# SidRama/Longitudinal-VAE

Measured on AMD Instinct MI355X. Metric: ELBO-steps/sec (exact-KL L-VAE step, Health-MNIST N=4096 L=16), higher is better.
Workload: dtype f16x3-split (fp32-equivalent)

## Files before the change

### longitudinal-vae_amd/csrc/kl_hyper.hip

```cpp
#include "blkinv.hpp"
#include "gram_tab.hpp"
#include "prof.hpp"

namespace lvae {

constexpr int kHbMaxBin = 4;
constexpr int kHbBins = 128;
constexpr int kHbBins2 = 4096;
constexpr int kHbRun = 64;
constexpr int kHbSmall = 16;
constexpr int kHbSmallest = 4;
constexpr int kHbNear = 4;
constexpr int kHbBlk = 4;
constexpr int kHbT = 64;
constexpr int kHbTP = 68;
constexpr int kHbNB = 24;
constexpr int kHbNQ = kHbNB / 4;
constexpr int kHbNearS = 2 * kHbBins2;
constexpr int kHbNearK = kHbNearS + kHbNear + 1;
constexpr int kHbA = kHbNearK + kHbNear;
constexpr int kHbTail = 2 * kHbNear + 1 + kHbBins;
constexpr int kHbPart = 2 * kHbBins2 + kHbTail;

struct HbDev {
  int on, nbin, big, nbins, nb2, nnear;
  int gmin[kTabMaxBits], grng[kTabMaxBits];
  int wmin[kTabMaxG], wrng[kTabMaxG];
  int bmask[kHbMaxBin], bgrp[kHbMaxBin], boff[kHbMaxBin], bn[kHbMaxBin], b2off[kHbMaxBin];
  int cbin[LVAE_MAX_COMP];
  int nslot[kHbNear];
};

typedef unsigned hb_u32x4 __attribute__((ext_vector_type(4)));

struct HbWs {
  HbDev* dev;
  uint8_t* pbin;
  int* rs;
  int* re;
  double* part;
  float* tab;
  hb_u32x4* rkey;
  double* hscr;
  double* nscr;
  size_t bytes;
  HbWs(char* base, int np_, int L) {
    size_t off = 0;
    auto take = [&](size_t b) {
      char* p = base ? base + off : nullptr;
      off += align256(b);
      return p;
    };
    dev = (HbDev*)take(sizeof(HbDev));
    pbin = (uint8_t*)take((size_t)kHbMaxBin * np_);
    rs = (int*)take((size_t)np_ * sizeof(int));
    re = (int*)take((size_t)np_ * sizeof(int));
    part = (double*)take((size_t)L * (np_ / kHbT) * kHbPart * sizeof(double));
    tab = (float*)take((size_t)L * kTabMaxBwdLds * sizeof(float));
    rkey = (hb_u32x4*)take((size_t)np_ * sizeof(hb_u32x4));
    hscr = (double*)take((size_t)L * (np_ / kHbT) * kHbBins * kHbT * sizeof(double));
    nscr = (double*)take((size_t)L * (np_ / kHbT) * kHbNB * 256 * sizeof(double));
    bytes = off;
  }
};
size_t kl_hyper_bytes(int np_, int L) { return HbWs(nullptr, np_, L).bytes; }
HbDev* kl_hyper_dev(void* base, int np_, int L) { return HbWs((char*)base, np_, L).dev; }

__global__ __launch_bounds__(1024) void hb_plan_kernel(GramTab tb, const double* __restrict__ x, int ldx, int n,
                                                       int np_, const int* __restrict__ covflag, HbWs ws, int enable) {
  __shared__ int lo[kTabMaxBits + kTabMaxG], hi[kTabMaxBits + kTabMaxG];
  __shared__ int fail;
  __shared__ HbDev d;
  const int tid = threadIdx.x, nd = tb.nbits + tb.ng;
  if (*covflag != 2) {
    if (tid == 0) ws.dev->on = 0;
    return;
  }
  if (tid < kTabMaxBits + kTabMaxG) {
    lo[tid] = INT_MAX;
    hi[tid] = INT_MIN;
  }
  if (tid == 0) fail = 0;
  __syncthreads();
  for (int q = 0; q < nd; ++q) {
    const int dim = q < tb.nbits ? tb.bdim[q] : tb.gdim[q - tb.nbits];
    if (dim < 0) continue;
    int mn = INT_MAX, mx = INT_MIN;
    for (int i = tid; i < n; i += 1024) {
      const int v = (int)x[(int64_t)i * ldx + dim];
      mn = min(mn, v);
      mx = max(mx, v);
    }
#pragma unroll
    for (int o = 32; o > 0; o >>= 1) {
      mn = min(mn, __shfl_xor(mn, o, 64));
      mx = max(mx, __shfl_xor(mx, o, 64));
    }
    if ((tid & 63) == 0) {
      atomicMin(&lo[q], mn);
      atomicMax(&hi[q], mx);
    }
  }
  __syncthreads();
  if (tid == 0) {
    HbDev p{};
    int f = 0;
    p.big = -1;
    for (int b = 0; b < tb.nbits; ++b) {
      p.gmin[b] = lo[b];
      p.grng[b] = hi[b] - lo[b] + 1;
      if (tb.bkind[b] == LVAE_CAT && p.grng[b] > kHbSmallest && (p.big < 0 || p.grng[b] > p.grng[p.big])) p.big = b;
    }
    for (int b = 0; b < tb.nbits; ++b)
      if (b != p.big && tb.bkind[b] == LVAE_CAT && p.grng[b] > kHbSmall) f = 1;
    for (int g = 0; g < tb.ng; ++g) {
      p.wmin[g] = tb.gdim[g] >= 0 ? lo[tb.nbits + g] : 0;
      p.wrng[g] = tb.gdim[g] >= 0 ? hi[tb.nbits + g] - lo[tb.nbits + g] + 1 : 1;
    }
    for (int r = 0; r < tb.n_comp; ++r) {
      p.cbin[r] = -1;
      if (p.big >= 0 && ((tb.cmask[r] >> p.big) & 1)) continue;
      const int grp = tb.ckind[r] >= 0 ? tb.cgrp[r] : -1;
      int g = 0;
      while (g < p.nbin && !(p.bmask[g] == tb.cmask[r] && p.bgrp[g] == grp)) ++g;
      if (g == p.nbin) {
        if (p.nbin == kHbMaxBin) {
          f = 1;
          break;
        }
        long long nb = grp >= 0 ? p.wrng[grp] : 1;
        for (int b = 0; b < tb.nbits; ++b)
          if ((tb.cmask[r] >> b) & 1) nb *= p.grng[b];
        if (nb > kHbBins) {
          f = 1;
          break;
        }
        p.bmask[g] = tb.cmask[r];
        p.bgrp[g] = grp;
        p.bn[g] = (int)nb;
        p.boff[g] = p.nbins;
        p.b2off[g] = p.nb2;
        p.nbins += (int)nb;
        p.nb2 += (int)(nb * nb);
        ++p.nbin;
      }
      p.cbin[r] = g;
    }
    if (p.nbins > kHbBins || p.nb2 > kHbBins2) f = 1;
    {
      int nblk = 0;
      for (int g = 0; g < p.nbin; ++g) nblk += (p.bn[g] + 31) / 32;
      if (nblk > kHbBlk) f = 1;
    }
    for (int k = 0; k < tb.pbeg[tb.ng] && !f; ++k)
      if (p.cbin[tb.pcomp[tb.porder[k]]] < 0) {
        if (p.nnear == kHbNear) f = 1;
        else p.nslot[p.nnear++] = k;
      }
    d = p;
    fail = f;
  }
  __syncthreads();
  const int bd = d.big >= 0 ? tb.bdim[d.big] : -1;
  int bad = 0;
  for (int i = tid; i < np_; i += 1024) {
    int s = -1, e = -1;
    if (bd >= 0 && i < n) {
      const double v = x[(int64_t)i * ldx + bd];
      if (i > 0 && x[(int64_t)(i - 1) * ldx + bd] > v) bad = 1;
      s = i;
      while (s > 0 && i - s < kHbRun && x[(int64_t)(s - 1) * ldx + bd] == v) --s;
      e = i + 1;
      while (e < n && e - i < kHbRun && x[(int64_t)e * ldx + bd] == v) ++e;
      if (e - s > kHbRun || (s > 0 && x[(int64_t)(s - 1) * ldx + bd] == v) || (e < n && x[(int64_t)e * ldx + bd] == v))
        bad = 1;
    }
    ws.rs[i] = s;
    ws.re[i] = e;
    hb_u32x4 key = {0u, 0u, 0u, 0u};
    if (i < n) {
      for (int b = 0; b < tb.nbits; ++b) {
        const int xv = (int)x[(int64_t)i * ldx + tb.bdim[b]], v = xv - d.gmin[b];
        if (b == d.big) continue;
        if (tb.bkind[b] == LVAE_CAT) {
          if (v < 0 || v > 63) bad = 1;
          key.x |= (unsigned)(v & 63) << (6 * b);
        } else {
          if (xv != 0 && xv != 1) bad = 1;
          key.w |= (unsigned)(xv == 1) << b;
        }
      }
      for (int g = 0; g < tb.ng; ++g) {
        if (tb.gdim[g] < 0) continue;
        const int v = (int)x[(int64_t)i * ldx + tb.gdim[g]] - d.wmin[g];
        if (v < 0 || v > 65535) bad = 1;
        const unsigned u = (unsigned)(v & 0xffff);
        if (g == 0) key.y |= u;
        else if (g == 1) key.y |= u << 16;
        else key.z |= u;
      }
    }
    ws.rkey[i] = key;
    for (int g = 0; g < kHbMaxBin; ++g) {
      int idx = 255;
      if (g < d.nbin && i < n) {
        idx = 0;
        for (int b = 0; b < tb.nbits; ++b)
          if ((d.bmask[g] >> b) & 1) idx = idx * d.grng[b] + ((int)x[(int64_t)i * ldx + tb.bdim[b]] - d.gmin[b]);
        if (d.bgrp[g] >= 0) idx = idx * d.wrng[d.bgrp[g]] + ((int)x[(int64_t)i * ldx + tb.gdim[d.bgrp[g]]] - d.wmin[d.bgrp[g]]);
      }
      ws.pbin[(size_t)g * np_ + i] = (uint8_t)idx;
    }
  }
  if (__any(bad) && (tid & 63) == 0) atomicOr(&fail, 1);
  __syncthreads();
  if (tid == 0) {
    HbDev p = d;
    p.on = (!fail && enable) ? 1 : 0;
    *ws.dev = p;
  }
}


__global__ __launch_bounds__(256) void hb_tab_kernel(GramTab tb, HbWs ws, const double* __restrict__ params) {
  __shared__ float sp[64];
  const int tid = threadIdx.x, l = blockIdx.y, e = blockIdx.x * 256 + tid;
  if (!ws.dev->on) return;
  if (tid < tb.n_params) sp[tid] = float(params[(int64_t)l * tb.n_params + tid]);
  __syncthreads();
  if (e < tb.pbeg[tb.ng] * (1 << tb.nbits) * kTabR) ws.tab[(int64_t)l * kTabMaxBwdLds + e] = tab_bwd_entry(tb, sp, e);
}

__device__ inline unsigned hb_pair_code(hb_u32x4 ki, hb_u32x4 kj, unsigned catbits, int ng) {
  const unsigned x = ki.x ^ kj.x, x1 = x | (x >> 1), x3 = x1 | (x1 >> 2), x5 = x3 | (x1 >> 4);
  const unsigned fail = (((x5 & 0x1041041u) * 0x108421u) >> 20) & 31u;
  unsigned c = (catbits & ~fail) | (ki.w & kj.w);
  const unsigned a0 = ki.y & 0xffffu, b0 = kj.y & 0xffffu, a1 = ki.y >> 16, b1 = kj.y >> 16;
  const unsigned a2 = ki.z & 0xffffu, b2 = kj.z & 0xffffu;
  const unsigned d0 = a0 > b0 ? a0 - b0 : b0 - a0, d1 = a1 > b1 ? a1 - b1 : b1 - a1, d2 = a2 > b2 ? a2 - b2 : b2 - a2;
  const unsigned cap = (unsigned)kTabD;
  c |= (d0 < cap ? d0 : cap) << 8;
  if (ng > 1) c |= (d1 < cap ? d1 : cap) << 16;
  if (ng > 2) c |= (d2 < cap ? d2 : cap) << 24;
  return c;
}

__device__ inline unsigned hb_catbits(const GramTab& tb) {
  unsigned m = 0;
#pragma unroll
  for (int b = 0; b < kTabMaxBits; ++b)
    if (b < tb.nbits && tb.bkind[b] == LVAE_CAT) m |= 1u << b;
  return m;
}

__device__ inline void hb_near_tables(const GramTab& tb, const HbDev& d, const float* __restrict__ gt, int tstride,
                                      float* __restrict__ tab, int* __restrict__ sgrp) {
  const int tid = threadIdx.x;
  if (tid < d.nnear) sgrp[tid] = tb.cgrp[tb.pcomp[tb.porder[d.nslot[tid]]]];
  for (int e = tid; e < d.nnear * tstride; e += blockDim.x) tab[e] = gt[d.nslot[e / tstride] * tstride + e % tstride];
}

__device__ inline float hb_near_d(const float* tab, int tk, unsigned code, int grp) {
  return tab[tk + (int)(code & 0xffu) * kTabR + (int)((code >> (8 * (grp + 1))) & 0xffu)];
}

__global__ __launch_bounds__(256) void hb_near_kernel(GramTab tb, HbWs ws, int n, int np_,
                                                      const float* __restrict__ Kinv, const double* __restrict__ alpha) {
  __shared__ HbDev d;
  __shared__ int sgrp[kHbNear];
  __shared__ double red[4][kHbNear];
  extern __shared__ float ntab[];
  const int tid = threadIdx.x, lane = tid & 63, w = tid >> 6, I = blockIdx.x, l = blockIdx.y, I0 = I * kHbT;
  if (tid == 0) d = *ws.dev;
  __syncthreads();
  if (!d.on) return;
  const int tstride = (1 << tb.nbits) * kTabR, nnear = d.nnear;
  hb_near_tables(tb, d, ws.tab + (int64_t)l * kTabMaxBwdLds, tstride, ntab, sgrp);
  __syncthreads();
  const float* K = Kinv + (int64_t)l * np_ * np_;
  const double* al = alpha + (int64_t)l * np_;
  const unsigned catbits = hb_catbits(tb);
  double acc[kHbNear];
#pragma unroll
  for (int k = 0; k < kHbNear; ++k) acc[k] = 0.0;
  if (d.big >= 0) {
    for (int e = tid; e < kHbT * kHbRun; e += 256) {
      const int i = I0 + e / kHbRun, jj = e % kHbRun;
      if (i >= n) continue;
      const int s = ws.rs[i], len = ws.re[i] - s;
      if (jj >= len) continue;
      const int j = s + jj;
      const unsigned c = hb_pair_code(ws.rkey[i], ws.rkey[j], catbits, tb.ng);
      const double val = 0.5 * ((double)K[(int64_t)i * np_ + j] - al[i] * al[j]);
#pragma unroll
      for (int k = 0; k < kHbNear; ++k)
        if (k < nnear) acc[k] += val * (double)hb_near_d(ntab, k * tstride, c, sgrp[k]);
    }
  }
#pragma unroll
  for (int k = 0; k < kHbNear; ++k) {
    const double sk = wave_sum(acc[k]);
    if (lane == 0) red[w][k] = sk;
  }
  __syncthreads();
  if (tid < kHbNear)
    ws.part[((int64_t)l * (np_ / kHbT) + I) * kHbPart + kHbNearK + tid] =
        ((red[0][tid] + red[1][tid]) + red[2][tid]) + red[3][tid];
}


#ifdef LVAE_HB_STAMP
#define HB_STAMP(t)                                                                   \
  do {                                                                                \
    __builtin_amdgcn_sched_barrier(0);                                                \
    asm volatile("s_memtime %0\n\ts_waitcnt lgkmcnt(0)" : "=s"(t)::"memory");       \
    __builtin_amdgcn_sched_barrier(0);                                                \
  } while (0)
#else
#define HB_STAMP(t) \
  do {              \
  } while (0)
#endif

typedef float hb_f32x2 __attribute__((ext_vector_type(2)));
typedef float hb_f32x4 __attribute__((ext_vector_type(4)));
typedef float hb_f32x16 __attribute__((ext_vector_type(16)));
typedef __bf16 hb_bf16x8 __attribute__((ext_vector_type(8)));
typedef __bf16 hb_bf16x2 __attribute__((ext_vector_type(2)));
constexpr int kHbSlabThreads = 256, kHbSlabWaves = kHbSlabThreads / 64;
#ifndef LVAE_HB_FOLD
#define LVAE_HB_FOLD 16
#endif
constexpr int kHbFold = LVAE_HB_FOLD;
#ifndef LVAE_HB_DEPTH
#define LVAE_HB_DEPTH 1
#endif
constexpr int kHbDepth = LVAE_HB_DEPTH;
static_assert(kHbDepth == 1 || kHbDepth == 2 || kHbDepth == 4, "nt = np / 64 is a multiple of 4");

struct HbPre {
  hb_f32x2 pk[8];
  int pbn;
  hb_f32x4 vr[2];
};

__device__ inline unsigned hb_pk_bf16(float a, float b) {
  const hb_bf16x2 v = {(__bf16)a, (__bf16)b};
  return __builtin_bit_cast(unsigned, v);
}
__device__ inline float hb_bf_lo(unsigned u) { return __uint_as_float(u << 16); }
__device__ inline float hb_bf_hi(unsigned u) { return __uint_as_float(u & 0xffff0000u); }

__device__ inline int hb_pl_off(int c, int k) { return c * 32 + ((k ^ ((c >> 1) & 7)) << 2); }

__device__ inline void hb_split8(const float* a, hb_u32x4& hi, hb_u32x4& mid, hb_u32x4& lo) {
#pragma unroll
  for (int k = 0; k < 4; ++k) {
    const float x0 = a[2 * k], x1 = a[2 * k + 1];
    const unsigned h = hb_pk_bf16(x0, x1);
    const float r0 = x0 - hb_bf_lo(h), r1 = x1 - hb_bf_hi(h);
    const unsigned m = hb_pk_bf16(r0, r1);
    const float s0 = r0 - hb_bf_lo(m), s1 = r1 - hb_bf_hi(m);
    hi[k] = h;
    mid[k] = m;
    lo[k] = hb_pk_bf16(s0, s1);
  }
}

__global__ __launch_bounds__(kHbSlabThreads, 2) void hb_slab_kernel(GramTab tb, HbWs ws, int n, int np_,
                                                                    const float* __restrict__ Kinv,
                                                                    const float* __restrict__ vv,
                                                                    const double* __restrict__ alpha) {
  __shared__ HbDev d;
  __shared__ __attribute__((aligned(16))) float Tc[2 * kHbT * kHbTP];
  __shared__ __attribute__((aligned(16))) unsigned Pw[3][kHbT * 32];
  __shared__ __attribute__((aligned(8))) uint8_t rbin[kHbMaxBin][kHbT];
  __shared__ uint8_t cbin[kHbMaxBin][kHbT];
  __shared__ float vs[kHbT];
  __shared__ double acol[kHbT];
  __shared__ hb_u32x4 ckey[2 * kHbT];
  __shared__ int rstart[kHbT];
  __shared__ unsigned long long runends;
  __shared__ int nblk, nspan;
  __shared__ uint8_t blist[kHbNB];
  __shared__ int8_t blkid[64];
  __shared__ int sgrp[kHbNear];
  __shared__ int sbg[kHbBlk], sbb[kHbBlk], nbk;
  __shared__ double red[kHbSlabWaves][kHbNear + 1];
  extern __shared__ float tab[];
  const int tid = threadIdx.x, lane = tid & 63, w = tid >> 6, J = blockIdx.x, l = blockIdx.y, J0 = J * kHbT;
  if (tid == 0) d = *ws.dev;
  __syncthreads();
  if (!d.on) return;
  const int tstride = (1 << tb.nbits) * kTabR;
  if (tid < kHbT) {
    vs[tid] = vv[(int64_t)l * np_ + J0 + tid];
    acol[tid] = alpha[(int64_t)l * np_ + J0 + tid];
  }
  for (int e = tid; e < d.nbin * kHbT; e += kHbSlabThreads)
    cbin[e / kHbT][e % kHbT] = ws.pbin[(size_t)(e / kHbT) * np_ + J0 + e % kHbT];
  hb_near_tables(tb, d, ws.tab + (int64_t)l * kTabMaxBwdLds, tstride, tab, sgrp);
  if (tid < 2 * kHbT) {
    const int c = J0 - kHbT + tid;
    ckey[tid] = c >= 0 ? ws.rkey[c] : hb_u32x4{0u, 0u, 0u, 0u};
  }
  if (w == 0) {
    const int c = J0 + lane;
    const bool isend = d.big >= 0 && c < n && ws.re[c] == c + 1;
    const int s0 = isend ? ws.rs[c] : c;
    rstart[lane] = s0;
    const int ba = (s0 - J0 + kHbT) >> 4, bz = (c - J0 + kHbT) >> 4;
    unsigned long long m = 0;
    if (isend)
      for (int bi = ba; bi <= bz; ++bi)
        for (int bj = ba; bj <= bi; ++bj) m |= 1ull << (bi * 8 + bj);
#pragma unroll
    for (int o = 32; o > 0; o >>= 1) {
      const unsigned lo = __shfl_xor((unsigned)m, o, 64), hi = __shfl_xor((unsigned)(m >> 32), o, 64);
      m |= ((unsigned long long)hi << 32) | lo;
    }
    const unsigned long long ends = __ballot(isend), sp = __ballot(isend && s0 < J0);
    if (lane == 0) {
      runends = ends;
      nspan = sp != 0;
      int t = 0;
      for (int b = 0; b < 64; ++b) {
        blkid[b] = -1;
        if (((m >> b) & 1ull) && t < kHbNB) {
          blkid[b] = (int8_t)t;
          blist[t++] = (uint8_t)b;
        }
      }
      nblk = t;
    }
  }
  if (tid == 0) {
    int t = 0;
    for (int g = 0; g < d.nbin; ++g)
      for (int bb = 0; bb * 32 < d.bn[g] && t < kHbBlk; ++bb, ++t) {
        sbg[t] = g;
        sbb[t] = bb;
      }
    nbk = t;
  }
  __syncthreads();
  const float* K = Kinv + (int64_t)l * np_ * np_;
  const int nbin = d.nbin, nnear = d.nnear, nitem = 2 * nbk, nbl = nblk, span = nspan;
  const unsigned catbits = hb_catbits(tb);
  const int cb = w & 1, hh = lane >> 5, col = 32 * cb + (lane & 31);
  const int i0 = w, i1 = w + kHbSlabWaves;
  const bool it0 = i0 < nitem, it1 = i1 < nitem;
  int g0 = 0, b00 = 0, g1 = 0, b01 = 0;
  if (it0) {
    g0 = sbg[i0 >> 1];
    b00 = 32 * sbb[i0 >> 1];
  }
  if (it1) {
    g1 = sbg[i1 >> 1];
    b01 = 32 * sbb[i1 >> 1];
  }
  hb_f32x16 acc0 = {}, acc1 = {};
  double* Hs = ws.hscr + ((int64_t)l * (np_ / kHbT) + J) * kHbBins * kHbT;
  double* Ns = ws.nscr + ((int64_t)l * (np_ / kHbT) + J) * kHbNB * 256;
  const int li = lane & 15, lk = lane >> 4;
  bi_f32x4 nac[kHbNQ];
#pragma unroll
  for (int q = 0; q < kHbNQ; ++q) nac[q] = bi_f32x4{0.f, 0.f, 0.f, 0.f};
  double tS = 0.0;
  const int cp = tid & 31, i8 = tid >> 5;
  const float v0 = vs[2 * cp], v1 = vs[2 * cp + 1], r0 = sqrtf(v0), r1 = sqrtf(v1);
  const int nt = np_ / kHbT;

  auto fetch = [&](int I, HbPre& p) {
    const int I0 = I * kHbT;
#pragma unroll
    for (int u = 0; u < 8; ++u)
      p.pk[u] = __builtin_nontemporal_load(
          reinterpret_cast<const hb_f32x2*>(K + (int64_t)(I0 + 8 * i8 + u) * np_ + J0 + 2 * cp));
    p.pbn = (int)ws.pbin[(size_t)(w < nbin ? w : 0) * np_ + I0 + lane];
    const float* vr = vv + (int64_t)l * np_ + I0 + 8 * i8;
    p.vr[0] = *reinterpret_cast<const hb_f32x4*>(vr);
    p.vr[1] = *reinterpret_cast<const hb_f32x4*>(vr + 4);
  };

  auto fold = [&](hb_f32x16& acc, int g, int b0, bool first) {
    const int nb = d.bn[g];
    double* hc = Hs + (int64_t)d.boff[g] * kHbT + col;
#pragma unroll
    for (int e = 0; e < 16; ++e) {
      const int b = b0 + (e & 3) + 8 * (e >> 2) + 4 * hh;
      if (b < nb) {
        if (first) hc[b * kHbT] = (double)acc[e];
        else unsafeAtomicAdd(hc + b * kHbT, (double)acc[e]);
      }
      acc[e] = 0.f;
    }
  };

  auto body = [&](int I, HbPre& p) {
    const int I0 = I * kHbT;
    const bool fold_now = (I & (kHbFold - 1)) == kHbFold - 1 || I == nt - 1, fold_first = I < kHbFold;
    {
      float ts = 0.f;
#pragma unroll
      for (int u = 0; u < 8; ++u) {
        const float s0 = p.pk[u][0] * r0, s1 = p.pk[u][1] * r1;
        ts += s0 * s0 + s1 * s1;
      }
      tS += (double)ts;
#pragma unroll
      for (int c = 0; c < 2; ++c) {
        float a[8];
#pragma unroll
        for (int u = 0; u < 8; ++u) a[u] = p.pk[u][c];
        hb_u32x4 hi, mid, lo;
        hb_split8(a, hi, mid, lo);
        const int off = hb_pl_off(2 * cp + c, i8);
        *reinterpret_cast<hb_u32x4*>(&Pw[0][off]) = hi;
        *reinterpret_cast<hb_u32x4*>(&Pw[1][off]) = mid;
        *reinterpret_cast<hb_u32x4*>(&Pw[2][off]) = lo;
      }
    }
    if (w < nbin) rbin[w][lane] = (uint8_t)p.pbn;
    if (nbl > 0) {
      float sr[8];
#pragma unroll
      for (int u = 0; u < 8; ++u) sr[u] = sqrtf(p.vr[u >> 2][u & 3]);
#pragma unroll
      for (int c = 0; c < 2; ++c) {
        float* dst = &Tc[(kHbT + 2 * cp + c) * kHbTP + 8 * i8];
        *reinterpret_cast<hb_f32x4*>(dst) = hb_f32x4{p.pk[0][c] * sr[0], p.pk[1][c] * sr[1], p.pk[2][c] * sr[2],
                                                     p.pk[3][c] * sr[3]};
        *reinterpret_cast<hb_f32x4*>(dst + 4) = hb_f32x4{p.pk[4][c] * sr[4], p.pk[5][c] * sr[5],
                                                         p.pk[6][c] * sr[6], p.pk[7][c] * sr[7]};
      }
      if (span) {
        hb_f32x2 q[8];
#pragma unroll
        for (int u = 0; u < 8; ++u)
          q[u] = *reinterpret_cast<const hb_f32x2*>(K + (int64_t)(I0 + 8 * i8 + u) * np_ + J0 - kHbT + 2 * cp);
#pragma unroll
        for (int c = 0; c < 2; ++c) {
          float* dst = &Tc[(2 * cp + c) * kHbTP + 8 * i8];
          *reinterpret_cast<hb_f32x4*>(dst) = hb_f32x4{q[0][c] * sr[0], q[1][c] * sr[1], q[2][c] * sr[2],
                                                       q[3][c] * sr[3]};
          *reinterpret_cast<hb_f32x4*>(dst + 4) = hb_f32x4{q[4][c] * sr[4], q[5][c] * sr[5], q[6][c] * sr[6],
                                                           q[7][c] * sr[7]};
        }
      }
    }
    __syncthreads();
    fetch(I + kHbDepth < nt ? I + kHbDepth : nt - 1, p);
    if (it0) {
      auto onehot = [&](int g, int b0, int ks) {
        const unsigned mybin = (unsigned)(b0 + (lane & 31));
        const uint2 rb = *reinterpret_cast<const uint2*>(&rbin[g][16 * ks + 8 * hh]);
        hb_u32x4 a;
#pragma unroll
        for (int k = 0; k < 4; ++k) {
          const unsigned wd = k < 2 ? rb.x : rb.y, sh = 16 * (k & 1);
          const unsigned lo_ = ((wd >> sh) & 0xffu) == mybin ? 0x3f80u : 0u;
          const unsigned hi_ = ((wd >> (sh + 8)) & 0xffu) == mybin ? 0x3f800000u : 0u;
          a[k] = lo_ | hi_;
        }
        return __builtin_bit_cast(hb_bf16x8, a);
      };
#pragma unroll
      for (int ks = 0; ks < 4; ++ks) {
        const hb_bf16x8 bh = *reinterpret_cast<const hb_bf16x8*>(&Pw[0][hb_pl_off(col, 2 * ks + hh)]);
        const hb_bf16x8 bm = *reinterpret_cast<const hb_bf16x8*>(&Pw[1][hb_pl_off(col, 2 * ks + hh)]);
        const hb_bf16x8 bl = *reinterpret_cast<const hb_bf16x8*>(&Pw[2][hb_pl_off(col, 2 * ks + hh)]);
        const hb_bf16x8 a0 = onehot(g0, b00, ks);
        acc0 = __builtin_amdgcn_mfma_f32_32x32x16_bf16(a0, bl, acc0, 0, 0, 0);
        acc0 = __builtin_amdgcn_mfma_f32_32x32x16_bf16(a0, bm, acc0, 0, 0, 0);
        acc0 = __builtin_amdgcn_mfma_f32_32x32x16_bf16(a0, bh, acc0, 0, 0, 0);
        if (it1) {
          const hb_bf16x8 a1 = onehot(g1, b01, ks);
          acc1 = __builtin_amdgcn_mfma_f32_32x32x16_bf16(a1, bl, acc1, 0, 0, 0);
          acc1 = __builtin_amdgcn_mfma_f32_32x32x16_bf16(a1, bm, acc1, 0, 0, 0);
          acc1 = __builtin_amdgcn_mfma_f32_32x32x16_bf16(a1, bh, acc1, 0, 0, 0);
        }
      }
      if (fold_now) {
        fold(acc0, g0, b00, fold_first);
        if (it1) fold(acc1, g1, b01, fold_first);
      }
    }
#pragma unroll
    for (int q = 0; q < kHbNQ; ++q) {
      const int t = w + kHbSlabWaves * q;
      if (t < nbl) {
        const int bb = blist[t], bi = bb >> 3, bj = bb & 7;
        const float* pa = &Tc[(16 * bi + li) * kHbTP + 16 * lk];
        const float* pb = &Tc[(16 * bj + li) * kHbTP + 16 * lk];
        hb_f32x4 a4[4], b4[4];
#pragma unroll
        for (int s4 = 0; s4 < 4; ++s4) {
          a4[s4] = *reinterpret_cast<const hb_f32x4*>(pa + 4 * s4);
          b4[s4] = *reinterpret_cast<const hb_f32x4*>(pb + 4 * s4);
        }
        bi_f32x4 x0 = {0.f, 0.f, 0.f, 0.f}, x1 = {0.f, 0.f, 0.f, 0.f};
#pragma unroll
        for (int s4 = 0; s4 < 4; ++s4) {
          x0 = __builtin_amdgcn_mfma_f32_16x16x4f32(a4[s4][0], b4[s4][0], x0, 0, 0, 0);
          x1 = __builtin_amdgcn_mfma_f32_16x16x4f32(a4[s4][1], b4[s4][1], x1, 0, 0, 0);
          x0 = __builtin_amdgcn_mfma_f32_16x16x4f32(a4[s4][2], b4[s4][2], x0, 0, 0, 0);
          x1 = __builtin_amdgcn_mfma_f32_16x16x4f32(a4[s4][3], b4[s4][3], x1, 0, 0, 0);
        }
        nac[q] += x0 + x1;
        if (fold_now) {
          double* nb = Ns + t * 256 + (4 * lk) * 16 + li;
#pragma unroll
          for (int e = 0; e < 4; ++e) {
            if (fold_first) nb[e * 16] = (double)nac[q][e];
            else unsafeAtomicAdd(nb + e * 16, (double)nac[q][e]);
          }
          nac[q] = bi_f32x4{0.f, 0.f, 0.f, 0.f};
        }
      }
    }
    __syncthreads();
  };

  HbPre pre[kHbDepth];
#pragma unroll
  for (int u = 0; u < kHbDepth; ++u) fetch(u, pre[u]);
  for (int I = 0; I < nt; I += kHbDepth) {
#pragma unroll
    for (int u = 0; u < kHbDepth; ++u) body(I + u, pre[u]);
  }
  __builtin_amdgcn_s_waitcnt(0);
  __threadfence_block();
  __syncthreads();
  double* Qs = reinterpret_cast<double*>(&Tc[0]);
  for (int e = tid; e < d.nb2; e += kHbSlabThreads) Qs[e] = 0.0;
  __syncthreads();
  double* out = ws.part + ((int64_t)l * nt + J) * kHbPart;
  for (int tb2 = tid; tb2 < d.nbins; tb2 += kHbSlabThreads) {
    int g = 0;
    while (g + 1 < nbin && tb2 >= d.boff[g + 1]) ++g;
    const int b = tb2 - d.boff[g], nb = d.bn[g];
    double* qrow = Qs + d.b2off[g] + b * nb;
    const double* hr = Hs + (int64_t)tb2 * kHbT;
    double as = 0.0;
    for (int m = 0; m < kHbT; ++m) {
      const int bc = cbin[g][m];
      if (bc != 255) qrow[bc] += hr[m];
      if (bc == b) as += acol[m];
    }
    out[kHbA + tb2] = as;
  }
  __syncthreads();
  for (int e = tid; e < d.nb2; e += kHbSlabThreads) out[kHbBins2 + e] = Qs[e];
  for (int g = 0; g < nbin; ++g) {
    const int nb = d.bn[g], nb16 = (nb + 15) >> 4;
    for (int item = w; item < nb16 * nb16; item += kHbSlabWaves) {
      const int bi = item / nb16, bj = item % nb16, li = lane & 15, lk = lane >> 4;
      const int ba = 16 * bi + li, bb = 16 * bj + li;
      const double* ha = Hs + (int64_t)(d.boff[g] + (ba < nb ? ba : 0)) * kHbT;
      const double* hb = Hs + (int64_t)(d.boff[g] + (bb < nb ? bb : 0)) * kHbT;
      bi_f64x4 acc = {0.0, 0.0, 0.0, 0.0};
#pragma unroll 4
      for (int s4 = 0; s4 < kHbT; s4 += 4) {
        const int m = s4 + lk;
        const double a = ba < nb ? ha[m] * (double)vs[m] : 0.0;
        const double b = bb < nb ? hb[m] : 0.0;
        acc = __builtin_amdgcn_mfma_f64_16x16x4f64(a, b, acc, 0, 0, 0);
      }
#pragma unroll
      for (int q = 0; q < 4; ++q) {
        const int r = 16 * bi + lk + 4 * q, c = 16 * bj + li;
        if (r < nb && c < nb) out[d.b2off[g] + r * nb + c] = acc[q];
      }
    }
  }
  double nacc[kHbNear];
#pragma unroll
  for (int k = 0; k < kHbNear; ++k) nacc[k] = 0.0;
  for (unsigned long long rm = runends; rm; rm &= rm - 1) {
    const int e = __builtin_ctzll(rm), s0 = rstart[e], len = e + 1 - (s0 - J0);
    for (int pq = tid; pq < len * len; pq += kHbSlabThreads) {
      const int wi = s0 - J0 + kHbT + pq / len, wj = s0 - J0 + kHbT + pq % len;
      const int lo_ = min(wi, wj), hi_ = max(wi, wj);
      const int t = blkid[((hi_ >> 4) << 3) | (lo_ >> 4)];
      const double sv = t >= 0 ? Ns[t * 256 + (hi_ & 15) * 16 + (lo_ & 15)] : 0.0;
      const unsigned c = hb_pair_code(ckey[wi], ckey[wj], catbits, tb.ng);
      const int cb8 = (int)(c & 0xffu) * kTabR;
#pragma unroll
      for (int k2 = 0; k2 < kHbNear; ++k2) {
        if (k2 >= nnear) break;
        const int g = sgrp[k2];
        nacc[k2] += sv * (double)tab[k2 * tstride + cb8 + (int)((c >> (8 * (g + 1))) & 0xffu)];
      }
    }
  }
#pragma unroll
  for (int k = 0; k < kHbNear; ++k) {
    const double sk = wave_sum(nacc[k]);
    if (lane == 0) red[w][k] = sk;
  }
  {
    const double st = wave_sum(tS);
    if (lane == 0) red[w][kHbNear] = st;
  }
  __syncthreads();
  if (tid <= kHbNear) {
    double t = 0.0;
#pragma unroll
    for (int u = 0; u < kHbSlabWaves; ++u) t += red[u][tid];
    out[kHbNearS + tid] = t;
  }
}

constexpr int kNoiseSlotHb = 64, kBwdSlotsHb = 65;

__global__ __launch_bounds__(256) void hb_sum_kernel(HbWs ws, int np_) {
  const int i = blockIdx.x * 256 + threadIdx.x, l = blockIdx.y, nt = np_ / kHbT, nb2 = ws.dev->nb2;
  if (!ws.dev->on || i >= 2 * nb2 + kHbTail) return;
  const int e = i < nb2 ? i : i < 2 * nb2 ? kHbBins2 + i - nb2 : 2 * kHbBins2 + i - 2 * nb2;
  double* pl = ws.part + (int64_t)l * nt * kHbPart + e;
  double s = 0.0;
#pragma unroll 16
  for (int J = 0; J < nt; ++J) s += pl[(int64_t)J * kHbPart];
  pl[0] = s;
}

__global__ __launch_bounds__(256) void hb_final_kernel(GramTab tb, HbWs ws, int n, int np_,
                                                       const double* __restrict__ alpha,
                                                       const double* __restrict__ kdiag, double* __restrict__ part,
                                                       int G) {
  __shared__ HbDev d;
  __shared__ double Gb[kHbBins2];
  __shared__ double raw[kBwdSlotsHb];
  __shared__ double red[4];
  __shared__ double nz;
  extern __shared__ float ftab[];
  const int tid = threadIdx.x, lane = tid & 63, w = tid >> 6, l = blockIdx.x, nt = np_ / kHbT;
  if (tid == 0) d = *ws.dev;
  __syncthreads();
  if (!d.on) return;
  if (tid < kBwdSlotsHb) raw[tid] = 0.0;
  const double* al = alpha + (int64_t)l * np_;
  const double* pl = ws.part + (int64_t)l * nt * kHbPart;
  {
    const float* gt = ws.tab + (int64_t)l * kTabMaxBwdLds;
    for (int e = tid; e < tb.pbeg[tb.ng] * (1 << tb.nbits) * kTabR; e += 256) ftab[e] = gt[e];
  }
  for (int e = tid; e < d.nb2; e += 256) {
    int g = 0;
    while (g + 1 < d.nbin && e >= d.b2off[g + 1]) ++g;
    const int nb = d.bn[g], b = (e - d.b2off[g]) / nb, bc = (e - d.b2off[g]) % nb;
    const double m = pl[e], q = pl[kHbBins2 + e];
    Gb[e] = 0.5 * (q - m - pl[kHbA + d.boff[g] + b] * pl[kHbA + d.boff[g] + bc]);
  }
  {
    double s = 0.0;
    for (int i = tid; i < n; i += 256) s += kdiag[(int64_t)l * np_ + i] - al[i] * al[i];
    s = wave_sum(s);
    if (lane == 0) red[w] = s;
  }
  __syncthreads();
  if (tid == 0) {
    nz = 0.5 * ((((red[0] + red[1]) + red[2]) + red[3]) - pl[kHbNearS + kHbNear]);
    for (int k = 0; k < d.nnear; ++k)
      raw[tb.porder[d.nslot[k]]] = -0.5 * pl[kHbNearS + k] + pl[kHbNearK + k];
  }
  const int tstride = (1 << tb.nbits) * kTabR;
  for (int k = 0; k < tb.pbeg[tb.ng]; ++k) {
    const int p = tb.porder[k], r = tb.pcomp[p], g = d.cbin[r];
    if (g < 0) continue;
    const int nb = d.bn[g], grp = d.bgrp[g], W = grp >= 0 ? d.wrng[grp] : 1;
    double s = 0.0;
    for (int e = tid; e < nb * nb; e += 256) {
      int b = e / nb, bc = e % nb;
      const int w1 = b % W, w2 = bc % W;
      b /= W;
      bc /= W;
      int bits = 0;
#pragma unroll
      for (int q = kTabMaxBits - 1; q >= 0; --q) {
        if (q >= tb.nbits || !((d.bmask[g] >> q) & 1)) continue;
        const int v1 = b % d.grng[q] + d.gmin[q], v2 = bc % d.grng[q] + d.gmin[q];
        b /= d.grng[q];
        bc /= d.grng[q];
        const bool pass = tb.bkind[q] == LVAE_CAT ? v1 == v2 : v1 + v2 == 2;
        bits += pass ? (kTabR << q) : 0;
      }
      s += Gb[d.b2off[g] + e] * (double)ftab[k * tstride + bits + abs(w1 - w2)];
    }
    s = wave_sum(s);
    __syncthreads();
    if (lane == 0) red[w] = s;
    __syncthreads();
    if (tid == 0) raw[p] = ((red[0] + red[1]) + red[2]) + red[3];
  }
  __syncthreads();
  if (tid == 0) raw[kNoiseSlotHb] = nz;
  __syncthreads();
  for (int e = tid; e < kBwdSlotsHb * G; e += 256) {
    const int slot = e / G, gg = e % G;
    part[((int64_t)l * kBwdSlotsHb + slot) * G + gg] = gg == 0 ? raw[slot] : 0.0;
  }
}

static int hb_enabled() {
  const char* v = getenv("LVAE_KL_HYPER");
  return !v || atoi(v) != 0;
}

static size_t hb_slab_lds(const GramTab& tb) {
  static size_t stat = 0;
  if (!stat) {
    hipFuncAttributes a;
    if (hipFuncGetAttributes(&a, reinterpret_cast<const void*>(&hb_slab_kernel)) != hipSuccess) return 0;
    stat = a.sharedSizeBytes;
  }
  const int ns = tb.pbeg[tb.ng] < kHbNear ? tb.pbeg[tb.ng] : kHbNear;
  const size_t dyn = (size_t)ns * (1 << tb.nbits) * kTabR * sizeof(float);
  return stat + dyn <= 160 * 1024 ? (dyn ? dyn : 4) : 0;
}

static bool hb_host_ok(const lvae_kernel_spec* spec, GramTab& tb) {
  return gram_tab_build(spec, tb) && hb_enabled() && hb_slab_lds(tb) > 0;
}

int kl_hyper_plan(const lvae_kernel_spec* spec, const double* x, int ldx, int n, int np_, int L, void* wsbase,
                  const int* covflag, hipStream_t st) {
  HbWs ws((char*)wsbase, np_, L);
  GramTab tb;
  if (!hb_host_ok(spec, tb)) {
    if (zero_async(ws.dev, sizeof(HbDev), st) != 0) return LVAE_ERR_LAUNCH;
    return 0;
  }
  hb_plan_kernel<<<1, 1024, 0, st>>>(tb, x, ldx, n, np_, covflag, ws, 1);
  LVAE_CHECK_LAUNCH();
  return 0;
}

int kl_hyper_bwd(const lvae_kernel_spec* spec, const double* x, int ldx, int n, int np_, int L, const double* params,
                 const float* Kinv, const float* v, const double* alpha, const double* kdiag, void* wsbase, double* part,
                 int G, hipStream_t st) {
  (void)x;
  (void)ldx;
  HbWs ws((char*)wsbase, np_, L);
  GramTab tb;
  if (!gram_tab_build(spec, tb) || hb_slab_lds(tb) == 0) return 0;
  const size_t tabb = (size_t)tb.pbeg[tb.ng] * (1 << tb.nbits) * kTabR * sizeof(float);
  const size_t sdyn = hb_slab_lds(tb), ndyn = sdyn;
  const int nt = np_ / kHbT;
  hb_tab_kernel<<<dim3((unsigned)((tabb / sizeof(float) + 255) / 256), L), 256, 0, st>>>(tb, ws, params);
  hb_near_kernel<<<dim3(nt, L), 256, ndyn, st>>>(tb, ws, n, np_, Kinv, alpha);
  {
    ProfScope ps(LVAE_PH_HB_SLAB, st);
    hb_slab_kernel<<<dim3(nt, L), kHbSlabThreads, sdyn, st>>>(tb, ws, n, np_, Kinv, v, alpha);
  }
  hb_sum_kernel<<<dim3((2 * kHbBins2 + kHbTail + 255) / 256, L), 256, 0, st>>>(ws, np_);
  hb_final_kernel<<<L, 256, tabb, st>>>(tb, ws, n, np_, alpha, kdiag, part, G);
  LVAE_CHECK_LAUNCH();
  return 0;
}

}

extern "C" int lvae_kl_closed_hyper_state(int n, int L, const void* workspace, int32_t* on, void* stream) {
  if (n <= 0) return -1;
  if (L <= 0) return -2;
  if (!workspace) return -3;
  if (!on) return -4;
  size_t kl_hyper_offset_in_kl_ws(int np_, int L);
  const int np_ = (n + 255) / 256 * 256;
  const char* hb = (const char*)workspace + kl_hyper_offset_in_kl_ws(np_, L);
  const lvae::HbWs ws(const_cast<char*>(hb), np_, L);
  if (lvae::copy_words_async(on, &ws.dev->on, sizeof(int32_t), (hipStream_t)stream) != 0) return LVAE_ERR_LAUNCH;
  return 0;
}
```

Before: 123.8.

## Split hyper-KL slab kernel over row segments and move epilogue to separate kernel

The slab kernel now launches an extra grid dimension of row segments, each covering kHbFold tiles. Each segment writes its partial histogram and near-block accumulators as fp32 to per-segment scratch, replacing the per-fold fp64 atomic adds into one buffer. A new epilogue kernel sums the segments in double, reduces the per-tile trace terms, and runs the Q/alpha and MFMA f64 post-processing with register-prefetched loads. This adds parallelism for small grids and removes atomics and the serial tail from the slab kernel, at the cost of an extra launch, more scratch memory and extra global traffic.

```diff
diff --git a/longitudinal-vae_amd/csrc/kl_hyper.hip b/longitudinal-vae_amd/csrc/kl_hyper.hip
--- a/longitudinal-vae_amd/csrc/kl_hyper.hip
+++ b/longitudinal-vae_amd/csrc/kl_hyper.hip
@@ -22,6 +22,13 @@
 constexpr int kHbTail = 2 * kHbNear + 1 + kHbBins;
 constexpr int kHbPart = 2 * kHbBins2 + kHbTail;
 
+#ifndef LVAE_HB_FOLD
+#define LVAE_HB_FOLD 16
+#endif
+constexpr int kHbFold = LVAE_HB_FOLD;
+constexpr int kHbSlabThreads = 256, kHbSlabWaves = kHbSlabThreads / 64;
+constexpr int hb_nseg(int nt) { return (nt + kHbFold - 1) / kHbFold; }
+
 struct HbDev {
   int on, nbin, big, nbins, nb2, nnear;
   int gmin[kTabMaxBits], grng[kTabMaxBits];
@@ -41,8 +48,11 @@
   double* part;
   float* tab;
   hb_u32x4* rkey;
-  double* hscr;
-  double* nscr;
+  float* hscr;
+  float* nscr;
+  double* hsum;
+  double* nsum;
+  float* tscr;
   size_t bytes;
   HbWs(char* base, int np_, int L) {
     size_t off = 0;
@@ -58,8 +68,12 @@
     part = (double*)take((size_t)L * (np_ / kHbT) * kHbPart * sizeof(double));
     tab = (float*)take((size_t)L * kTabMaxBwdLds * sizeof(float));
     rkey = (hb_u32x4*)take((size_t)np_ * sizeof(hb_u32x4));
-    hscr = (double*)take((size_t)L * (np_ / kHbT) * kHbBins * kHbT * sizeof(double));
-    nscr = (double*)take((size_t)L * (np_ / kHbT) * kHbNB * 256 * sizeof(double));
+    const size_t nt = np_ / kHbT, R = hb_nseg((int)nt);
+    hscr = (float*)take((size_t)L * nt * R * kHbBins * kHbT * sizeof(float));
+    nscr = (float*)take((size_t)L * nt * R * kHbNB * 256 * sizeof(float));
+    hsum = (double*)take((size_t)L * nt * kHbBins * kHbT * sizeof(double));
+    nsum = (double*)take((size_t)L * nt * kHbNB * 256 * sizeof(double));
+    tscr = (float*)take((size_t)L * nt * nt * kHbSlabThreads * sizeof(float));
     bytes = off;
   }
 };
@@ -327,16 +341,12 @@
 typedef float hb_f32x16 __attribute__((ext_vector_type(16)));
 typedef __bf16 hb_bf16x8 __attribute__((ext_vector_type(8)));
 typedef __bf16 hb_bf16x2 __attribute__((ext_vector_type(2)));
-constexpr int kHbSlabThreads = 256, kHbSlabWaves = kHbSlabThreads / 64;
-#ifndef LVAE_HB_FOLD
-#define LVAE_HB_FOLD 16
-#endif
-constexpr int kHbFold = LVAE_HB_FOLD;
 #ifndef LVAE_HB_DEPTH
 #define LVAE_HB_DEPTH 1
 #endif
 constexpr int kHbDepth = LVAE_HB_DEPTH;
 static_assert(kHbDepth == 1 || kHbDepth == 2 || kHbDepth == 4, "nt = np / 64 is a multiple of 4");
+static_assert(kHbFold >= 4 && (kHbFold & (kHbFold - 1)) == 0, "a segment is a whole number of prefetch rotations");
 
 struct HbPre {
   hb_f32x2 pk[8];
@@ -367,74 +377,51 @@
   }
 }
 
-__global__ __launch_bounds__(kHbSlabThreads, 2) void hb_slab_kernel(GramTab tb, HbWs ws, int n, int np_,
+__device__ inline void hb_run_scan(const HbDev& d, const HbWs& ws, int n, int J0, int lane, int* rstart,
+                                   unsigned long long* runends, int* nspan, int* nblk, uint8_t* blist,
+                                   int8_t* blkid) {
+  const int c = J0 + lane;
+  const bool isend = d.big >= 0 && c < n && ws.re[c] == c + 1;
+  const int s0 = isend ? ws.rs[c] : c;
+  if (rstart) rstart[lane] = s0;
+  const int ba = (s0 - J0 + kHbT) >> 4, bz = (c - J0 + kHbT) >> 4;
+  unsigned long long m = 0;
+  if (isend)
+    for (int bi = ba; bi <= bz; ++bi)
+      for (int bj = ba; bj <= bi; ++bj) m |= 1ull << (bi * 8 + bj);
+#pragma unroll
+  for (int o = 32; o > 0; o >>= 1) {
+    const unsigned lo = __shfl_xor((unsigned)m, o, 64), hi = __shfl_xor((unsigned)(m >> 32), o, 64);
+    m |= ((unsigned long long)hi << 32) | lo;
+  }
+  const unsigned long long ends = __ballot(isend), sp = __ballot(isend && s0 < J0);
+  const int t = __popcll(m & ((1ull << lane) - 1ull));
+  const bool mine = ((m >> lane) & 1ull) && t < kHbNB;
+  if (blkid) blkid[lane] = mine ? (int8_t)t : (int8_t)-1;
+  if (blist && mine) blist[t] = (uint8_t)lane;
+  if (lane == 0) {
+    if (runends) *runends = ends;
+    if (nspan) *nspan = sp != 0;
+    if (nblk) *nblk = min(__popcll(m), kHbNB);
+  }
+}
+
+__global__ __launch_bounds__(kHbSlabThreads, 2) void hb_slab_kernel(HbWs ws, int n, int np_,
                                                                     const float* __restrict__ Kinv,
-                                                                    const float* __restrict__ vv,
-                                                                    const double* __restrict__ alpha) {
+                                                                    const float* __restrict__ vv) {
   __shared__ HbDev d;
   __shared__ __attribute__((aligned(16))) float Tc[2 * kHbT * kHbTP];
   __shared__ __attribute__((aligned(16))) unsigned Pw[3][kHbT * 32];
   __shared__ __attribute__((aligned(8))) uint8_t rbin[kHbMaxBin][kHbT];
-  __shared__ uint8_t cbin[kHbMaxBin][kHbT];
-  __shared__ float vs[kHbT];
-  __shared__ double acol[kHbT];
-  __shared__ hb_u32x4 ckey[2 * kHbT];
-  __shared__ int rstart[kHbT];
-  __shared__ unsigned long long runends;
   __shared__ int nblk, nspan;
   __shared__ uint8_t blist[kHbNB];
-  __shared__ int8_t blkid[64];
-  __shared__ int sgrp[kHbNear];
   __shared__ int sbg[kHbBlk], sbb[kHbBlk], nbk;
-  __shared__ double red[kHbSlabWaves][kHbNear + 1];
-  extern __shared__ float tab[];
   const int tid = threadIdx.x, lane = tid & 63, w = tid >> 6, J = blockIdx.x, l = blockIdx.y, J0 = J * kHbT;
   if (tid == 0) d = *ws.dev;
   __syncthreads();
   if (!d.on) return;
-  const int tstride = (1 << tb.nbits) * kTabR;
-  if (tid < kHbT) {
-    vs[tid] = vv[(int64_t)l * np_ + J0 + tid];
-    acol[tid] = alpha[(int64_t)l * np_ + J0 + tid];
-  }
-  for (int e = tid; e < d.nbin * kHbT; e += kHbSlabThreads)
-    cbin[e / kHbT][e % kHbT] = ws.pbin[(size_t)(e / kHbT) * np_ + J0 + e % kHbT];
-  hb_near_tables(tb, d, ws.tab + (int64_t)l * kTabMaxBwdLds, tstride, tab, sgrp);
-  if (tid < 2 * kHbT) {
-    const int c = J0 - kHbT + tid;
-    ckey[tid] = c >= 0 ? ws.rkey[c] : hb_u32x4{0u, 0u, 0u, 0u};
-  }
-  if (w == 0) {
-    const int c = J0 + lane;
-    const bool isend = d.big >= 0 && c < n && ws.re[c] == c + 1;
-    const int s0 = isend ? ws.rs[c] : c;
-    rstart[lane] = s0;
-    const int ba = (s0 - J0 + kHbT) >> 4, bz = (c - J0 + kHbT) >> 4;
-    unsigned long long m = 0;
-    if (isend)
-      for (int bi = ba; bi <= bz; ++bi)
-        for (int bj = ba; bj <= bi; ++bj) m |= 1ull << (bi * 8 + bj);
-#pragma unroll
-    for (int o = 32; o > 0; o >>= 1) {
-      const unsigned lo = __shfl_xor((unsigned)m, o, 64), hi = __shfl_xor((unsigned)(m >> 32), o, 64);
-      m |= ((unsigned long long)hi << 32) | lo;
-    }
-    const unsigned long long ends = __ballot(isend), sp = __ballot(isend && s0 < J0);
-    if (lane == 0) {
-      runends = ends;
-      nspan = sp != 0;
-      int t = 0;
-      for (int b = 0; b < 64; ++b) {
-        blkid[b] = -1;
-        if (((m >> b) & 1ull) && t < kHbNB) {
-          blkid[b] = (int8_t)t;
-          blist[t++] = (uint8_t)b;
-        }
-      }
-      nblk = t;
-    }
-  }
-  if (tid == 0) {
+  if (w == 0) hb_run_scan(d, ws, n, J0, lane, nullptr, nullptr, &nspan, &nblk, blist, nullptr);
+  if (tid == 64) {
     int t = 0;
     for (int g = 0; g < d.nbin; ++g)
       for (int bb = 0; bb * 32 < d.bn[g] && t < kHbBlk; ++bb, ++t) {
@@ -445,8 +432,7 @@
   }
   __syncthreads();
   const float* K = Kinv + (int64_t)l * np_ * np_;
-  const int nbin = d.nbin, nnear = d.nnear, nitem = 2 * nbk, nbl = nblk, span = nspan;
-  const unsigned catbits = hb_catbits(tb);
+  const int nbin = d.nbin, nitem = 2 * nbk, nbl = nblk, span = nspan;
   const int cb = w & 1, hh = lane >> 5, col = 32 * cb + (lane & 31);
   const int i0 = w, i1 = w + kHbSlabWaves;
   const bool it0 = i0 < nitem, it1 = i1 < nitem;
@@ -460,16 +446,18 @@
     b01 = 32 * sbb[i1 >> 1];
   }
   hb_f32x16 acc0 = {}, acc1 = {};
-  double* Hs = ws.hscr + ((int64_t)l * (np_ / kHbT) + J) * kHbBins * kHbT;
-  double* Ns = ws.nscr + ((int64_t)l * (np_ / kHbT) + J) * kHbNB * 256;
+  const int nt = np_ / kHbT, R = hb_nseg(nt), seg = blockIdx.z, Ia = kHbFold * seg, Ib = min(Ia + kHbFold, nt);
+  const int64_t sj = (int64_t)l * nt + J;
+  float* Hs = ws.hscr + (sj * R + seg) * kHbBins * kHbT;
+  float* Ns = ws.nscr + (sj * R + seg) * kHbNB * 256;
+  float* Ts = ws.tscr + sj * nt * kHbSlabThreads + tid;
   const int li = lane & 15, lk = lane >> 4;
   bi_f32x4 nac[kHbNQ];
 #pragma unroll
   for (int q = 0; q < kHbNQ; ++q) nac[q] = bi_f32x4{0.f, 0.f, 0.f, 0.f};
-  double tS = 0.0;
   const int cp = tid & 31, i8 = tid >> 5;
-  const float v0 = vs[2 * cp], v1 = vs[2 * cp + 1], r0 = sqrtf(v0), r1 = sqrtf(v1);
-  const int nt = np_ / kHbT;
+  const hb_f32x2 v01 = *reinterpret_cast<const hb_f32x2*>(vv + (int64_t)l * np_ + J0 + 2 * cp);
+  const float r0 = sqrtf(v01[0]), r1 = sqrtf(v01[1]);
 
   auto fetch = [&](int I, HbPre& p) {
     const int I0 = I * kHbT;
@@ -483,23 +471,18 @@
     p.vr[1] = *reinterpret_cast<const hb_f32x4*>(vr + 4);
   };
 
-  auto fold = [&](hb_f32x16& acc, int g, int b0, bool first) {
+  auto store_h = [&](const hb_f32x16& acc, int g, int b0) {
     const int nb = d.bn[g];
-    double* hc = Hs + (int64_t)d.boff[g] * kHbT + col;
+    float* hc = Hs + (int64_t)d.boff[g] * kHbT + col;
 #pragma unroll
     for (int e = 0; e < 16; ++e) {
       const int b = b0 + (e & 3) + 8 * (e >> 2) + 4 * hh;
-      if (b < nb) {
-        if (first) hc[b * kHbT] = (double)acc[e];
-        else unsafeAtomicAdd(hc + b * kHbT, (double)acc[e]);
-      }
-      acc[e] = 0.f;
+      if (b < nb) hc[b * kHbT] = acc[e];
     }
   };
 
   auto body = [&](int I, HbPre& p) {
     const int I0 = I * kHbT;
-    const bool fold_now = (I & (kHbFold - 1)) == kHbFold - 1 || I == nt - 1, fold_first = I < kHbFold;
     {
       float ts = 0.f;
 #pragma unroll
@@ -507,7 +490,7 @@
         const float s0 = p.pk[u][0] * r0, s1 = p.pk[u][1] * r1;
         ts += s0 * s0 + s1 * s1;
       }
-      tS += (double)ts;
+      Ts[I * kHbSlabThreads] = ts;
 #pragma unroll
       for (int c = 0; c < 2; ++c) {
         float a[8];
@@ -550,7 +533,7 @@
       }
     }
     __syncthreads();
-    fetch(I + kHbDepth < nt ? I + kHbDepth : nt - 1, p);
+    fetch(I + kHbDepth < Ib ? I + kHbDepth : Ib - 1, p);
     if (it0) {
       auto onehot = [&](int g, int b0, int ks) {
         const unsigned mybin = (unsigned)(b0 + (lane & 31));
@@ -581,10 +564,6 @@
           acc1 = __builtin_amdgcn_mfma_f32_32x32x16_bf16(a1, bh, acc1, 0, 0, 0);
         }
       }
-      if (fold_now) {
-        fold(acc0, g0, b00, fold_first);
-        if (it1) fold(acc1, g1, b01, fold_first);
-      }
     }
 #pragma unroll
     for (int q = 0; q < kHbNQ; ++q) {
@@ -608,15 +587,6 @@
           x1 = __builtin_amdgcn_mfma_f32_16x16x4f32(a4[s4][3], b4[s4][3], x1, 0, 0, 0);
         }
         nac[q] += x0 + x1;
-        if (fold_now) {
-          double* nb = Ns + t * 256 + (4 * lk) * 16 + li;
-#pragma unroll
-          for (int e = 0; e < 4; ++e) {
-            if (fold_first) nb[e * 16] = (double)nac[q][e];
-            else unsafeAtomicAdd(nb + e * 16, (double)nac[q][e]);
-          }
-          nac[q] = bi_f32x4{0.f, 0.f, 0.f, 0.f};
-        }
       }
     }
     __syncthreads();
@@ -624,18 +594,102 @@
 
   HbPre pre[kHbDepth];
 #pragma unroll
-  for (int u = 0; u < kHbDepth; ++u) fetch(u, pre[u]);
-  for (int I = 0; I < nt; I += kHbDepth) {
+  for (int u = 0; u < kHbDepth; ++u) fetch(Ia + u, pre[u]);
+  for (int I = Ia; I < Ib; I += kHbDepth) {
 #pragma unroll
     for (int u = 0; u < kHbDepth; ++u) body(I + u, pre[u]);
+  }
+  if (it0) {
+    store_h(acc0, g0, b00);
+    if (it1) store_h(acc1, g1, b01);
+  }
+#pragma unroll
+  for (int q = 0; q < kHbNQ; ++q) {
+    const int t = w + kHbSlabWaves * q;
+    if (t < nbl) {
+      float* nb = Ns + t * 256 + (4 * lk) * 16 + li;
+#pragma unroll
+      for (int e = 0; e < 4; ++e) nb[e * 16] = nac[q][e];
+    }
+  }
+}
+
+__global__ __launch_bounds__(kHbSlabThreads) void hb_epi_kernel(GramTab tb, HbWs ws, int n, int np_,
+                                                                const float* __restrict__ vv,
+                                                                const double* __restrict__ alpha) {
+  __shared__ HbDev d;
+  __shared__ double Qs[kHbBins2];
+  __shared__ uint8_t cbin[kHbMaxBin][kHbT];
+  __shared__ float vs[kHbT];
+  __shared__ double acol[kHbT];
+  __shared__ hb_u32x4 ckey[2 * kHbT];
+  __shared__ int rstart[kHbT];
+  __shared__ unsigned long long runends;
+  __shared__ int nblk;
+  __shared__ int8_t blkid[64];
+  __shared__ int sgrp[kHbNear];
+  __shared__ double red[kHbSlabWaves][kHbNear + 1];
+  extern __shared__ float tab[];
+  const int tid = threadIdx.x, lane = tid & 63, w = tid >> 6, J = blockIdx.x, l = blockIdx.y, J0 = J * kHbT;
+  if (tid == 0) d = *ws.dev;
+  __syncthreads();
+  if (!d.on) return;
+  const int tstride = (1 << tb.nbits) * kTabR;
+  if (tid < kHbT) {
+    vs[tid] = vv[(int64_t)l * np_ + J0 + tid];
+    acol[tid] = alpha[(int64_t)l * np_ + J0 + tid];
+  }
+  for (int e = tid; e < d.nbin * kHbT; e += kHbSlabThreads)
+    cbin[e / kHbT][e % kHbT] = ws.pbin[(size_t)(e / kHbT) * np_ + J0 + e % kHbT];
+  hb_near_tables(tb, d, ws.tab + (int64_t)l * kTabMaxBwdLds, tstride, tab, sgrp);
+  if (tid < 2 * kHbT) {
+    const int c = J0 - kHbT + tid;
+    ckey[tid] = c >= 0 ? ws.rkey[c] : hb_u32x4{0u, 0u, 0u, 0u};
+  }
+  if (w == 0) hb_run_scan(d, ws, n, J0, lane, rstart, &runends, nullptr, &nblk, nullptr, blkid);
+  for (int e = tid; e < d.nb2; e += kHbSlabThreads) Qs[e] = 0.0;
+  __syncthreads();
+  const int nbin = d.nbin, nnear = d.nnear, nt = np_ / kHbT, R = hb_nseg(nt);
+  const unsigned catbits = hb_catbits(tb);
+  const int64_t sj = (int64_t)l * nt + J;
+  double* Hs = ws.hsum + sj * kHbBins * kHbT;
+  double* Ns = ws.nsum + sj * kHbNB * 256;
+  {
+    auto sum_segs = [&](const float* __restrict__ src, double* __restrict__ dst, int count, int64_t stride) {
+      for (int e0 = tid; e0 < count; e0 += 4 * kHbSlabThreads) {
+        double s[4];
+#pragma unroll
+        for (int u = 0; u < 4; ++u) s[u] = (double)src[min(e0 + u * kHbSlabThreads, count - 1)];
+        for (int r = 1; r < R; ++r) {
+          float x[4];
+#pragma unroll
+          for (int u = 0; u < 4; ++u) x[u] = src[r * stride + min(e0 + u * kHbSlabThreads, count - 1)];
+#pragma unroll
+          for (int u = 0; u < 4; ++u) s[u] += (double)x[u];
+        }
+#pragma unroll
+        for (int u = 0; u < 4; ++u)
+          if (e0 + u * kHbSlabThreads < count) dst[e0 + u * kHbSlabThreads] = s[u];
+      }
+    };
+    sum_segs(ws.hscr + sj * R * kHbBins * kHbT, Hs, d.nbins * kHbT, (int64_t)kHbBins * kHbT);
+    sum_segs(ws.nscr + sj * R * kHbNB * 256, Ns, nblk * 256, (int64_t)kHbNB * 256);
+  }
+  double tS = 0.0;
+  {
+    const float* Ts = ws.tscr + sj * nt * kHbSlabThreads + tid;
+    for (int I = 0; I < nt; I += 4) {
+      float t4[4];
+#pragma unroll
+      for (int u = 0; u < 4; ++u) t4[u] = Ts[(I + u) * kHbSlabThreads];
+#pragma unroll
+      for (int u = 0; u < 4; ++u) tS += (double)t4[u];
+    }
   }
   __builtin_amdgcn_s_waitcnt(0);
   __threadfence_block();
   __syncthreads();
-  double* Qs = reinterpret_cast<double*>(&Tc[0]);
-  for (int e = tid; e < d.nb2; e += kHbSlabThreads) Qs[e] = 0.0;
-  __syncthreads();
-  double* out = ws.part + ((int64_t)l * nt + J) * kHbPart;
+  double* out = ws.part + sj * kHbPart;
   for (int tb2 = tid; tb2 < d.nbins; tb2 += kHbSlabThreads) {
     int g = 0;
     while (g + 1 < nbin && tb2 >= d.boff[g + 1]) ++g;
@@ -643,10 +697,16 @@
     double* qrow = Qs + d.b2off[g] + b * nb;
     const double* hr = Hs + (int64_t)tb2 * kHbT;
     double as = 0.0;
-    for (int m = 0; m < kHbT; ++m) {
-      const int bc = cbin[g][m];
-      if (bc != 255) qrow[bc] += hr[m];
-      if (bc == b) as += acol[m];
+    for (int m0 = 0; m0 < kHbT; m0 += 16) {
+      double h[16];
+#pragma unroll
+      for (int u = 0; u < 16; ++u) h[u] = hr[m0 + u];
+#pragma unroll
+      for (int u = 0; u < 16; ++u) {
+        const int m = m0 + u, bc = cbin[g][m];
+        if (bc != 255) qrow[bc] += h[u];
+        if (bc == b) as += acol[m];
+      }
     }
     out[kHbA + tb2] = as;
   }
@@ -660,11 +720,17 @@
       const double* ha = Hs + (int64_t)(d.boff[g] + (ba < nb ? ba : 0)) * kHbT;
       const double* hb = Hs + (int64_t)(d.boff[g] + (bb < nb ? bb : 0)) * kHbT;
       bi_f64x4 acc = {0.0, 0.0, 0.0, 0.0};
-#pragma unroll 4
-      for (int s4 = 0; s4 < kHbT; s4 += 4) {
-        const int m = s4 + lk;
-        const double a = ba < nb ? ha[m] * (double)vs[m] : 0.0;
-        const double b = bb < nb ? hb[m] : 0.0;
+      double ax[kHbT / 4], bx[kHbT / 4];
+#pragma unroll
+      for (int s = 0; s < kHbT / 4; ++s) {
+        ax[s] = ha[4 * s + lk];
+        bx[s] = hb[4 * s + lk];
+      }
+#pragma unroll
+      for (int s = 0; s < kHbT / 4; ++s) {
+        const int m = 4 * s + lk;
+        const double a = ba < nb ? ax[s] * (double)vs[m] : 0.0;
+        const double b = bb < nb ? bx[s] : 0.0;
         acc = __builtin_amdgcn_mfma_f64_16x16x4f64(a, b, acc, 0, 0, 0);
       }
 #pragma unroll
@@ -811,9 +877,10 @@
 static size_t hb_slab_lds(const GramTab& tb) {
   static size_t stat = 0;
   if (!stat) {
-    hipFuncAttributes a;
+    hipFuncAttributes a, b;
     if (hipFuncGetAttributes(&a, reinterpret_cast<const void*>(&hb_slab_kernel)) != hipSuccess) return 0;
-    stat = a.sharedSizeBytes;
+    if (hipFuncGetAttributes(&b, reinterpret_cast<const void*>(&hb_epi_kernel)) != hipSuccess) return 0;
+    stat = a.sharedSizeBytes > b.sharedSizeBytes ? a.sharedSizeBytes : b.sharedSizeBytes;
   }
   const int ns = tb.pbeg[tb.ng] < kHbNear ? tb.pbeg[tb.ng] : kHbNear;
   const size_t dyn = (size_t)ns * (1 << tb.nbits) * kTabR * sizeof(float);
@@ -852,7 +919,8 @@
   hb_near_kernel<<<dim3(nt, L), 256, ndyn, st>>>(tb, ws, n, np_, Kinv, alpha);
   {
     ProfScope ps(LVAE_PH_HB_SLAB, st);
-    hb_slab_kernel<<<dim3(nt, L), kHbSlabThreads, sdyn, st>>>(tb, ws, n, np_, Kinv, v, alpha);
+    hb_slab_kernel<<<dim3(nt, L, hb_nseg(nt)), kHbSlabThreads, 0, st>>>(ws, n, np_, Kinv, v);
+    hb_epi_kernel<<<dim3(nt, L), kHbSlabThreads, sdyn, st>>>(tb, ws, n, np_, v, alpha);
   }
   hb_sum_kernel<<<dim3((2 * kHbBins2 + kHbTail + 255) / 256, L), 256, 0, st>>>(ws, np_);
   hb_final_kernel<<<L, 256, tabb, st>>>(tb, ws, n, np_, alpha, kdiag, part, G);
```

Result: no change. 124.9, median of 6 (+0.9%).
